# HerreraKrachTeichmann/NJODE

Hardware: AMD Instinct MI355X
Metric: paths/sec (training step) on 20k Black-Scholes, 100 steps (higher is better)
Workload: dtype f32; 1 GPU; BlackScholes 20000 paths/GPU x 100 grid steps, every rank's paths as one batch, hidden_size=10, 3x(50,50) tanh nets, dropout 0.1, train step = plan+fwd+bwd+Adam; global_batch=20000, n_obs_rows=199470, euler_steps_per_batch=1820212, params=10071, parallelism=dp1

## Files before the change

njode_amd/csrc/njode_mfma.h:

```cpp
#pragma once
#include "njode_kernels.h"

namespace njode {

typedef float f32x4 __attribute__((ext_vector_type(4)));

NJ_DEV f32x4 mfma4(float a, float b, f32x4 c) {
  return __builtin_amdgcn_mfma_f32_16x16x4f32(a, b, c, 0, 0, 0);
}

typedef unsigned u32x2 __attribute__((ext_vector_type(2)));
NJ_DEV f32x4 mfma1(float a, float b, f32x4 c) {
  return __builtin_amdgcn_mfma_f32_4x4x1f32(a, b, c, 0, 0, 0);
}
NJ_DEV float edge_reduce(float p0, float p1) {
  const u32x2 s = __builtin_amdgcn_permlane16_swap(__float_as_uint(p0), __float_as_uint(p1), false, false);
  const float t = __uint_as_float(s[0]) + __uint_as_float(s[1]);
  const u32x2 w = __builtin_amdgcn_permlane32_swap(__float_as_uint(t), __float_as_uint(t), false, false);
  return __uint_as_float(w[0]) + __uint_as_float(w[1]);
}
template <int W> struct EdgeRows {
  static constexpr int R = (W % 16 == 1 || W % 16 == 2) ? W % 16 : 0;
  static constexpr int TILE = R ? W / 16 : -1;
};
// ... 140 lines not shown
    float v = act_f<ACT>(acc[q / 4][q % 4]);
    if constexpr (DROP) v = ((keep >> q) & 1) ? v * inv_keep : 0.0f;
    av[q] = v;
  }
  constexpr int QB = W / 4, GB = W % 4;
  av[QB] = g == GB ? 1.0f : av[QB];
}
template <class C, bool DROP>
NJ_DEV void hidden_from_acc(const f32x4 (&acc)[MF<C>::MT1], float (&av)[MF<C>::Q1], uint32_t keep,
                            float inv_keep, int g) {
  hidden_from_acc_g<MF<C>::MT1, MF<C>::Q1, MF<C>::W, C::ACT, DROP>(acc, av, keep, inv_keep, g);
}

template <class C, bool DROP>
NJ_DEV void hidden_from_acc_draw(const f32x4 (&acc)[MF<C>::MT1], float (&av)[MF<C>::Q1], uint32_t& s,
                                 uint32_t thr16, float inv_keep, int g) {
  constexpr int Q1 = MF<C>::Q1;
#pragma unroll
  for (int q = 0; q < Q1; q += 2) {
    float v0 = act_f<C::ACT>(acc[q / 4][q % 4]);
    float v1 = q + 1 < Q1 ? act_f<C::ACT>(acc[(q + 1) / 4][(q + 1) % 4]) : 0.0f;
    if constexpr (DROP) {
      s ^= s << 13; s ^= s >> 17; s ^= s << 5;
      v0 = (s & 0xffffu) >= thr16 ? v0 * inv_keep : 0.0f;
      v1 = (s >> 16) >= thr16 ? v1 * inv_keep : 0.0f;
    }
    av[q] = v0;
    if (q + 1 < Q1) av[q + 1] = v1;
  }
  constexpr int QB = MF<C>::W / 4, GB = MF<C>::W % 4;
  av[QB] = g == GB ? 1.0f : av[QB];
}

template <class C, bool DROP, bool TAIL>
NJ_DEV void ode_fwd_single(const KArgs& a, int lane, int wave, int n_waves, int tile0, int tile1) {
  using M = MF<C>;
  const int g = lane >> 4, c = lane & 15;
  float A1[M::MT1][M::Q0], A2[M::MT1][M::Q1], A3[M::MTH][M::Q1];
#pragma unroll
  for (int mt = 0; mt < M::MT1; ++mt) {
#pragma unroll
    for (int q = 0; q < M::Q0; ++q) A1[mt][q] = a.frag[(M::F1 + mt * M::Q0 + q) * 64 + lane];
#pragma unroll
    for (int q = 0; q < M::Q1; ++q) A2[mt][q] = a.frag[(M::F2 + mt * M::Q1 + q) * 64 + lane];
  }
#pragma unroll
  for (int mt = 0; mt < M::MTH; ++mt)
#pragma unroll
    for (int q = 0; q < M::Q1; ++q) A3[mt][q] = a.frag[(M::F3 + mt * M::Q1 + q) * 64 + lane];

  const bool SAVE = !TAIL && a.save_traj != 0;
  const int n_items = TAIL ? a.B : a.n_obs;
  const int n_tiles = tile1 - tile0;
  float* const trash = a.trash + lane * C::H;
  for (int round = 0; round * n_waves < n_tiles; ++round) {
    const int rel = snake_tile(round, wave, n_waves);
    if (rel >= n_tiles) continue;
    const int tile = tile0 + rel;
    const int j = tile * 16 + c;
    const bool valid = j < n_items;
    Item<C> it;
    it.template load<TAIL>(a, j, valid);
    const float* h0 = it.h0(a);
    float h[M::QH];
#pragma unroll
    for (int q = 0; q < M::QH; ++q) {
// ... 424 lines not shown
```

njode_amd/csrc/njode_mfma_rows.h:

```cpp
#pragma once
#include "njode_mfma.h"

namespace njode {

template <int IN_, int OUT_, int W_> struct MS {
  static constexpr int IN = IN_, OUT = OUT_, W = W_;
  static constexpr int Q0 = (IN + 1 + 3) / 4, Q1 = (W + 1 + 3) / 4;
  static constexpr int QO = (OUT + 3) / 4, QW = (W + 3) / 4, QI = (IN + 3) / 4;
  static constexpr int MT1 = (W + 15) / 16, MTO = (OUT + 15) / 16, MTI = (IN + 15) / 16;
  static constexpr int NT1 = (W + 1 + 15) / 16, NT0 = (IN + 1 + 15) / 16;
  static constexpr int F1 = 0, F2 = F1 + MT1 * Q0, F3 = F2 + MT1 * Q1, NFWD = F3 + MTO * Q1;
  static constexpr int B3 = NFWD, B2 = B3 + MT1 * QO, B1 = B2 + MT1 * QW, NALL = B1 + MTI * QW;
  static constexpr int ET = EdgeRows<W>::TILE, ER = EdgeRows<W>::R;
  static constexpr int G2M = ER ? ET : MT1, G2N = ER ? ET : NT1;
};

template <class NL, class S>
NJ_DEV void pack_net_value(const float* __restrict__ Pn, float* __restrict__ frag, int idx) {
  if (idx >= S::NALL * 64) return;
  const int f = idx >> 6, l = idx & 63, g = l >> 4, c = l & 15;
  const float *W1 = Pn + NL::woff(0), *b1 = Pn + NL::boff(0), *W2 = Pn + NL::woff(1),
              *b2 = Pn + NL::boff(1), *W3 = Pn + NL::woff(2), *b3 = Pn + NL::boff(2);
  float v = 0.0f;
  if (f < S::F2) {
// ... 32 lines not shown
      for (int q = 0; q < S::Q0; ++q) A1[mt][q] = frag[(S::F1 + mt * S::Q0 + q) * 64 + l];
#pragma unroll
      for (int q = 0; q < S::Q1; ++q) A2[mt][q] = frag[(S::F2 + mt * S::Q1 + q) * 64 + l];
    }
    const int l3 = S::OUT == 1 ? (lane & 48) : lane;
#pragma unroll
    for (int mt = 0; mt < S::MTO; ++mt)
#pragma unroll
      for (int q = 0; q < S::Q1; ++q) A3[mt][q] = frag[(S::F3 + mt * S::Q1 + q) * 64 + l3];
  }
  NJ_DEV float r3(int q) const { return A3[0][q]; }
  NJ_DEV void begin() const {}
  NJ_DEV float a1(int mt, int q) const { return A1[mt][q]; }
  NJ_DEV float a2(int mt, int q) const { return A2[mt][q]; }
  NJ_DEV float a3(int mt, int q) const { return A3[mt][q]; }
  NJ_DEV float e1(int q) const { return A1[S::ET < 0 ? 0 : S::ET][q]; }
  NJ_DEV float e2(int q) const { return A2[S::ET < 0 ? 0 : S::ET][q]; }
};
template <class S> struct LdsFrags {
  lfp base;
  lfp cur;
  int de;
  int dr;
  NJ_DEV void init(lfp img, int lane) {
    base = img + lane;
    cur = base;
    de = edge_lane(lane) - lane;
    dr = (lane & 48) - lane;
  }
  NJ_DEV float r3(int q) const { return cur[(S::F3 + q) * 64 + dr]; }
  static NJ_DEV void stage(lfp img, const float* frag, int tid, int nthreads) {
    for (int i = tid; i < S::NALL * 64; i += nthreads) img[i] = frag[i];
  }
  NJ_DEV void begin() {
    unsigned v = (unsigned)(unsigned long long)base;
    asm volatile("" : "+v"(v));
    cur = (lfp)(unsigned long long)v;
  }
  NJ_DEV float a1(int mt, int q) const { return cur[(S::F1 + mt * S::Q0 + q) * 64]; }
  NJ_DEV float a2(int mt, int q) const { return cur[(S::F2 + mt * S::Q1 + q) * 64]; }
  NJ_DEV float a3(int mt, int q) const { return cur[(S::F3 + mt * S::Q1 + q) * 64]; }
  NJ_DEV float b3(int mt, int q) const { return cur[(S::B3 + mt * S::QO + q) * 64]; }
  NJ_DEV float b2(int mt, int q) const { return cur[(S::B2 + mt * S::QW + q) * 64]; }
  NJ_DEV float b1(int mt, int q) const { return cur[(S::B1 + mt * S::QW + q) * 64]; }
  NJ_DEV float e1(int q) const { return cur[(S::F1 + S::ET * S::Q0 + q) * 64 + de]; }
  NJ_DEV float e2(int q) const { return cur[(S::F2 + S::ET * S::Q1 + q) * 64 + de]; }
  NJ_DEV float eb3(int q) const { return cur[(S::B3 + S::ET * S::QO + q) * 64 + de]; }
  NJ_DEV float eb2(int q) const { return cur[(S::B2 + S::ET * S::QW + q) * 64 + de]; }
};
template <class S> struct GradTiles {
  f32x4 G3[S::MTO][S::NT1], G2[S::G2M][S::G2N], GM[2], GN[2], G1[S::MT1][S::NT0];
  NJ_DEV void zero() {
    const f32x4 z = {0.f, 0.f, 0.f, 0.f};
    GM[0] = GM[1] = GN[0] = GN[1] = z;
#pragma unroll
    for (int i = 0; i < S::MTO; ++i)
#pragma unroll
      for (int n = 0; n < S::NT1; ++n) G3[i][n] = z;
#pragma unroll
    for (int i = 0; i < S::G2M; ++i)
#pragma unroll
      for (int n = 0; n < S::G2N; ++n) G2[i][n] = z;
#pragma unroll
    for (int i = 0; i < S::MT1; ++i) {
#pragma unroll
      for (int n = 0; n < S::NT0; ++n) G1[i][n] = z;
// ... 8 lines not shown
      for (int nt = 0; nt < S::NT1; ++nt) f(G3[mt][nt], i++);
#pragma unroll
    for (int mt = 0; mt < S::G2M; ++mt)
#pragma unroll
      for (int nt = 0; nt < S::G2N; ++nt) f(G2[mt][nt], i++);
    if constexpr (S::ER != 0) {
      f(GM[0], i++);
      f(GN[0], i++);
    }
#pragma unroll
    for (int mt = 0; mt < S::MT1; ++mt)
#pragma unroll
      for (int nt = 0; nt < S::NT0; ++nt) f(G1[mt][nt], i++);
  }
  NJ_DEV bool reduce_block(lfp lds, int wv, int lane) {
    f32x4 __attribute__((address_space(3)))* red = (f32x4 __attribute__((address_space(3)))*)lds;
    if constexpr (S::ER != 0) {
      const f32x4 z = {0.f, 0.f, 0.f, 0.f};
      GM[0] += GM[1];
      GN[0] += GN[1];
      GM[1] = GN[1] = z;
    }
    __syncthreads();
    if (wv > 0) for_tiles([&](f32x4& t, int i) { red[((wv - 1) * NG + i) * 64 + lane] = t; });
    __syncthreads();
    if (wv != 0) return false;
    for_tiles([&](f32x4& t, int i) {
      t += red[(0 * NG + i) * 64 + lane];
      t += red[(1 * NG + i) * 64 + lane];
      t += red[(2 * NG + i) * 64 + lane];
    });
    return true;
  }
  template <class NL> NJ_DEV void flush(float* slab, int g, int c) const {
    float *W1 = slab + NL::woff(0), *b1 = slab + NL::boff(0), *W2 = slab + NL::woff(1),
          *b2 = slab + NL::boff(1), *W3 = slab + NL::woff(2), *b3 = slab + NL::boff(2);
#pragma unroll
    for (int mt = 0; mt < S::G2M; ++mt)
#pragma unroll
      for (int r = 0; r < 4; ++r) {
        const int uo = 16 * mt + 4 * g + r;
        if (uo < S::W) {
#pragma unroll
          for (int nt = 0; nt < S::G2N; ++nt) {
            const int ui = 16 * nt + c;
            if (ui < S::W) W2[uo * S::W + ui] = G2[mt][nt][r];
            else if (ui == S::W) b2[uo] = G2[mt][nt][r];
          }
        }
      }
    if constexpr (S::ER != 0) {
      const int lane = 16 * g + c;
      const f32x4 gm = GM[0] + GM[1], gn = GN[0] + GN[1];
#pragma unroll
      for (int i = 0; i < S::ER; ++i) {
        const int uo = 16 * S::ET + i;
        if (lane < S::W) W2[uo * S::W + lane] = gm[i];
        else if (lane == S::W) b2[uo] = gm[i];
      }
      if (lane < 16 * S::ET) {
#pragma unroll
        for (int i = 0; i < 4; ++i) {
          const int ui = 16 * S::ET + i;
          if (ui < S::W) W2[lane * S::W + ui] = gn[i];
          else if (ui == S::W) b2[lane] = gn[i];
        }
// ... 14 lines not shown
        }
      }
    if constexpr (S::OUT == 1) {
#pragma unroll
      for (int q = 0; q < S::Q1; ++q) {
        float v = G3[0][q / 4][q % 4];
#pragma unroll
        for (int o = 8; o > 0; o >>= 1) v += __shfl_xor(v, o);
        const int ui = 4 * q + g;
        if (c == 0) {
          if (ui < S::W) W3[ui] = v;
          else if (ui == S::W) b3[0] = v;
        }
      }
      return;
    }
#pragma unroll
    for (int mt = 0; mt < S::MTO; ++mt)
#pragma unroll
      for (int r = 0; r < 4; ++r) {
        const int uo = 16 * mt + 4 * g + r;
        if (uo < S::OUT) {
#pragma unroll
          for (int nt = 0; nt < S::NT1; ++nt) {
            const int ui = 16 * nt + c;
            if (ui < S::W) W3[uo * S::W + ui] = G3[mt][nt][r];
            else if (ui == S::W) b3[uo] = G3[mt][nt][r];
          }
        }
      }
  }
};

template <class S, int ACT, bool DROP, class FP>
NJ_DEV void mnet_fwd(FP& F, const float (&b0)[S::Q0], float (&a1)[S::Q1],
                     float (&a2)[S::Q1], f32x4 (&out)[S::MTO], uint32_t k1, uint32_t k2,
                     float inv_keep, int g) {
  const f32x4 z = {0.f, 0.f, 0.f, 0.f};
  f32x4 acc[S::MT1];
  F.begin();
#pragma unroll
  for (int mt = 0; mt < S::MT1; ++mt) acc[mt] = z;
#pragma unroll
  for (int q = 0; q < S::Q0; ++q)
#pragma unroll
    for (int mt = 0; mt < S::MT1; ++mt)
      acc[mt] = mt == S::ET ? mfma1(F.e1(q), b0[q], acc[mt]) : mfma4(F.a1(mt, q), b0[q], acc[mt]);
  if constexpr (S::ER != 0) acc[S::ET] = edge_tile<S::ER>(acc[S::ET], g);
  hidden_from_acc_g<S::MT1, S::Q1, S::W, ACT, DROP>(acc, a1, k1, inv_keep, g);
#pragma unroll
  for (int mt = 0; mt < S::MT1; ++mt) acc[mt] = z;
#pragma unroll
  for (int q = 0; q < S::Q1; ++q)
#pragma unroll
    for (int mt = 0; mt < S::MT1; ++mt)
      acc[mt] = mt == S::ET ? mfma1(F.e2(q), a1[q], acc[mt]) : mfma4(F.a2(mt, q), a1[q], acc[mt]);
  if constexpr (S::ER != 0) acc[S::ET] = edge_tile<S::ER>(acc[S::ET], g);
  hidden_from_acc_g<S::MT1, S::Q1, S::W, ACT, DROP>(acc, a2, k2, inv_keep, g);
  if constexpr (S::OUT == 1) {
    float p0 = 0.0f, p1 = 0.0f;
#pragma unroll
    for (int q = 0; q < S::Q1; q += 2) {
      p0 = fmaf(F.r3(q), a2[q], p0);
      if (q + 1 < S::Q1) p1 = fmaf(F.r3(q + 1), a2[q + 1], p1);
    }
    const float p = p0 + p1;
    out[0] = f32x4{edge_reduce(p, p), 0.0f, 0.0f, 0.0f};
    return;
  }
#pragma unroll
  for (int mt = 0; mt < S::MTO; ++mt) out[mt] = z;
#pragma unroll
  for (int q = 0; q < S::Q1; ++q)
#pragma unroll
    for (int mt = 0; mt < S::MTO; ++mt) out[mt] = mfma4(F.a3(mt, q), a2[q], out[mt]);
}

template <class S, int ACT, bool DROP, bool DIN, class FP, int ROWS = IMG_ROWS>
NJ_DEV void mnet_bwd(FP& Bf, GradTiles<S>& G, lfp img_d, lfp img_a,
                     const float (&dout)[S::QO], const float (&b0)[S::Q0],
                     const float (&a1)[S::Q1], const float (&a2)[S::Q1], uint32_t k1,
                     uint32_t k2, float inv_keep, float keepf, f32x4 (&din)[DIN ? S::MTI : 1],
                     int g, int c) {
  static_assert(16 * S::NT1 <= ROWS && 16 * S::NT0 <= ROWS && 16 * S::MTO <= ROWS &&
                    16 * S::MT1 <= ROWS,
                "dW staging images hold at most ROWS units");
  const f32x4 z = {0.f, 0.f, 0.f, 0.f};
  f32x4 acc[S::MT1];
  Bf.begin();
  if constexpr (S::OUT == 1) {
    const float d0 = g == 0 ? dout[0] : 0.0f;
    const float dyc = edge_reduce(d0, d0);
#pragma unroll
    for (int mt = 0; mt < S::MT1; ++mt) acc[mt] = z;
#pragma unroll
    for (int q = 0; q < S::Q1; ++q) {
      G.G3[0][q / 4][q % 4] = fmaf(dyc, a2[q], G.G3[0][q / 4][q % 4]);
      if (q < S::QW) {
        const float w = Bf.r3(q);
        acc[q / 4][q % 4] = (4 * q + 3 < S::W || 4 * q + g < S::W) ? w * dyc : 0.0f;
      }
    }
  } else {
    img_write<S::QO>(img_d, dout, g, c);
    img_write<S::Q1>(img_a, a2, g, c);
    wave_lds_sync();
    dw_accumulate<S::MTO, S::NT1>(img_d, img_a, G.G3, g, c);
#pragma unroll
    for (int mt = 0; mt < S::MT1; ++mt) acc[mt] = z;
#pragma unroll
    for (int q = 0; q < S::QO; ++q)
#pragma unroll
      for (int mt = 0; mt < S::MT1; ++mt)
        acc[mt] = mt == S::ET ? mfma1(Bf.eb3(q), dout[q], acc[mt]) : mfma4(Bf.b3(mt, q), dout[q], acc[mt]);
    if constexpr (S::ER != 0) acc[S::ET] = edge_tile<S::ER>(acc[S::ET], g);
  }
  float d2[S::QW];
  hidden_delta_g<S::MT1, S::Q1, S::QW, ACT, DROP>(acc, a2, d2, k2, inv_keep, keepf);
  wave_lds_sync();
  img_write<S::QW>(img_d, d2, g, c);
  img_write<S::Q1>(img_a, a1, g, c);
  wave_lds_sync();
  if constexpr (S::ER != 0) dw_accumulate_edge<S::G2M>(img_d, img_a, G.G2, G.GM, G.GN, 16 * g + c, g, c);
  else dw_accumulate<S::G2M, S::G2N>(img_d, img_a, G.G2, g, c);
#pragma unroll
  for (int mt = 0; mt < S::MT1; ++mt) acc[mt] = z;
#pragma unroll
  for (int q = 0; q < S::QW; ++q)
#pragma unroll
    for (int mt = 0; mt < S::MT1; ++mt)
      acc[mt] = mt == S::ET ? mfma1(Bf.eb2(q), d2[q], acc[mt]) : mfma4(Bf.b2(mt, q), d2[q], acc[mt]);
  if constexpr (S::ER != 0) acc[S::ET] = edge_tile<S::ER>(acc[S::ET], g);
  float d1[S::QW];
  hidden_delta_g<S::MT1, S::Q1, S::QW, ACT, DROP>(acc, a1, d1, k1, inv_keep, keepf);
  wave_lds_sync();
  img_write<S::QW>(img_d, d1, g, c);
  img_write<S::Q0>(img_a, b0, g, c);
  wave_lds_sync();
  dw_accumulate<S::MT1, S::NT0>(img_d, img_a, G.G1, g, c);
  if constexpr (DIN) {
#pragma unroll
    for (int mt = 0; mt < S::MTI; ++mt) din[mt] = z;
#pragma unroll
    for (int q = 0; q < S::QW; ++q)
#pragma unroll
      for (int mt = 0; mt < S::MTI; ++mt) din[mt] = mfma4(Bf.b1(mt, q), d1[q], din[mt]);
  }
  wave_lds_sync();
}

template <bool DROP> NJ_DEV void row_keep_bits(const KArgs& a, unsigned long long gid, uint32_t tkey,
                                               uint32_t net, int g, int nq, uint32_t& k1,
                                               uint32_t& k2) {
  k1 = k2 = 0;
  if constexpr (DROP) {
    uint32_t st = drop_state(a.dc, (uint32_t)gid, (uint32_t)(gid >> 32) + 0x5bd1e995u * (g + 1),
                             tkey, net);
    k1 = keep_bits<16>(st, a.dc.thr16);
    k2 = keep_bits<16>(st, a.dc.thr16);
  }
  (void)nq;
}

template <int Q, int N> NJ_DEV float by_group(const float (&v)[N], int g) {
  const float e0 = 4 * Q + 0 < N ? v[4 * Q + 0 < N ? 4 * Q + 0 : 0] : 0.0f;
  const float e1 = 4 * Q + 1 < N ? v[4 * Q + 1 < N ? 4 * Q + 1 : 0] : 0.0f;
  const float e2 = 4 * Q + 2 < N ? v[4 * Q + 2 < N ? 4 * Q + 2 : 0] : 0.0f;
  const float e3 = 4 * Q + 3 < N ? v[4 * Q + 3 < N ? 4 * Q + 3 : 0] : 0.0f;
  return g == 0 ? e0 : (g == 1 ? e1 : (g == 2 ? e2 : e3));
}

template <int NQ, int N, int Q = 0>
NJ_DEV void fill_by_group(float (&dq)[NQ], const float (&v)[N], int g) {
  if constexpr (Q < NQ) {
    dq[Q] = by_group<Q, N>(v, g);
    fill_by_group<NQ, N, Q + 1>(dq, v, g);
  }
}

template <class C> struct EncS { using type = MS<C::ENC_IN, C::H, C::W>; };
template <class C> struct DecS { using type = MS<C::H, C::DO, C::W>; };

template <class C, class S>
NJ_DEV void enc_input(const float* xp, float (&b0)[S::Q0], int g) {
#pragma unroll
  for (int q = 0; q < S::Q0; ++q) {
    const int u = 4 * q + g;
    const float xv = xp[u < C::D ? u : 0];
    b0[q] = u < C::D ? tanh_f(xv) : (u == C::D ? 1.0f : 0.0f);
  }
}
template <class C> NJ_DEV float enc_residual(const float* xp, int u) {
  if constexpr (C::ENC_CASE == 1) {
    return xp[u % C::D];
  } else if constexpr (C::ENC_CASE == 2) {
    constexpr int mult = C::D / C::H;
    float s = 0.0f;
#pragma unroll
    for (int cc = 0; cc < mult; ++cc) s += xp[cc * C::H + (u < C::H ? u : 0)];
    return s * (1.0f / mult);
  } else {
    return 0.0f;
  }
}

template <class C, bool DROP>
__global__ void __launch_bounds__(64) k_encode_rows_mfma(KArgs a) {
  using S = typename EncS<C>::type;
  const int lane = threadIdx.x, g = lane >> 4, c = lane & 15;
  FwdFrags<S> F;
  F.load(a.frag_enc, lane);
  const int total = a.n_obs + a.B;
  const int n_tiles = (total + 15) / 16;
  float* const trash = a.trash + lane * C::H;
  for (int tile = blockIdx.x; tile < n_tiles; tile += gridDim.x) {
    const int t0 = tile * 16 + c;
    const bool valid = t0 < total;
    const int tid = valid ? t0 : 0;
    const bool is_row = tid < a.n_obs;
    const int b = is_row ? a.obs_idx[tid] : tid - a.n_obs;
    const float* xp = is_row ? a.X + (size_t)tid * C::D : a.start_X + (size_t)b * C::D;
    float b0[S::Q0], a1[S::Q1], a2[S::Q1];
    enc_input<C, S>(xp, b0, g);
    uint32_t k1, k2;
    row_keep_bits<DROP>(a, a.gid0 + b, is_row ? (uint32_t)a.k_jump[a.t_of_row[tid]] : TKEY_START,
                        NET_ENC, g, S::Q1, k1, k2);
    f32x4 out[S::MTO];
    mnet_fwd<S, C::ACT, DROP>(F, b0, a1, a2, out, k1, k2, a.dc.inv_keep, g);
    float* dstrow = valid ? (is_row ? a.h0row + (size_t)tid * C::H : a.h0start + (size_t)b * C::H)
                          : trash;
#pragma unroll
    for (int q = 0; q < S::QO; ++q) {
      const int u = 4 * q + g;
      const float v = out[q / 4][q % 4] + enc_residual<C>(xp, u < C::H ? u : 0);
      float* dst = u < C::H ? dstrow + u : trash;
      *dst = v;
    }
  }
}

template <class C, class S>
NJ_DEV void dec_input(const float* hp, float (&b0)[S::Q0], int g) {
#pragma unroll
  for (int q = 0; q < S::Q0; ++q) {
    const int u = 4 * q + g;
    const float hv = hp[u < C::H ? u : 0];
    b0[q] = u < C::H ? tanh_f(hv) : (u == C::H ? 1.0f : 0.0f);
  }
}
template <class C, class S>
NJ_DEV void dec_collect(lfp img, const f32x4 (&out)[S::MTO], const float* hp, float (&y)[C::DO],
                        int g, int c) {
  if constexpr (C::DO == 1) {
    float v = out[0][0];
    if constexpr (C::DEC_CASE == 1) {
      v += hp[0];
    } else if constexpr (C::DEC_CASE == 2) {
      float s = 0.0f;
#pragma unroll
      for (int cc = 0; cc < C::H; ++cc) s += hp[cc];
      v += s * (1.0f / C::H);
// ... 13 lines not shown
      v += hp[u % C::H];
    } else if constexpr (C::DEC_CASE == 2) {
      constexpr int mult = C::H / C::DO;
      float s = 0.0f;
#pragma unroll
      for (int cc = 0; cc < mult; ++cc) s += hp[cc * C::DO + u];
      v += s * (1.0f / mult);
    }
    y[u] = v;
  }
  wave_lds_sync();
}

template <class C, bool DROP>
__global__ void __launch_bounds__(64) k_jump_rows_mfma(KArgs a) {
  using S = typename DecS<C>::type;
  static_assert(C::DO <= 16, "row kernels hold the full readout vector per lane");
  __shared__ __attribute__((aligned(16))) float lds_raw[IMG_FLOATS];
  lfp img = (lfp)lds_raw;
  const int lane = threadIdx.x, g = lane >> 4, c = lane & 15;
  FwdFrags<S> F;
  F.load(a.frag_dec, lane);
  const int n_tiles = (a.n_obs + 15) / 16;
  for (int tile = blockIdx.x; tile < n_tiles; tile += gridDim.x) {
    const int r0 = tile * 16 + c;
    const bool valid = r0 < a.n_obs;
    const int r = valid ? r0 : 0;
    const int b = a.obs_idx[r];
    const unsigned long long gid = a.gid0 + b;
    const uint32_t tkey = (uint32_t)a.k_jump[a.t_of_row[r]];
    const float *he = a.h_end + (size_t)r * C::H, *h0 = a.h0row + (size_t)r * C::H;
    float b0[S::Q0], a1[S::Q1], a2[S::Q1], y[C::DO], ybj[C::DO], x[C::D], mask[C::D];
    f32x4 out[S::MTO];
    uint32_t k1, k2;
    dec_input<C, S>(he, b0, g);
    row_keep_bits<DROP>(a, gid, tkey, NET_DEC_BJ, g, S::Q1, k1, k2);
    mnet_fwd<S, C::ACT, DROP>(F, b0, a1, a2, out, k1, k2, a.dc.inv_keep, g);
    dec_collect<C, S>(img, out, he, ybj, g, c);
    dec_input<C, S>(h0, b0, g);
    row_keep_bits<DROP>(a, gid, tkey, NET_DEC, g, S::Q1, k1, k2);
    mnet_fwd<S, C::ACT, DROP>(F, b0, a1, a2, out, k1, k2, a.dc.inv_keep, g);
    dec_collect<C, S>(img, out, h0, y, g, c);
    load_vec(a.X + (size_t)r * C::D, x);
#pragma unroll
    for (int i = 0; i < C::D; ++i) mask[i] = 1.0f;
    float dy[C::DO], dybj[C::DO];
    const float scale = a.inv_batch * __builtin_amdgcn_rcpf((float)a.n_obs_ot[b]);
    const float term = loss_row<C>(x, mask, y, ybj, a.weight, a.loss_easy, scale, dy, dybj);
    if (valid && g == 0) a.loss_terms[r] = term;
  }
}

template <class C, class S>
NJ_DEV void dec_input_grad(const f32x4 (&din)[S::MTI], const float (&b0)[S::Q0],
                           const float (&dyv)[C::DO], float* dst, float* trash, int g) {
#pragma unroll
  for (int q = 0; q < S::QI; ++q) {
    const int u = 4 * q + g;
    const float th = b0[q];
    float v = din[q / 4][q % 4] * (1.0f - th * th);
    if constexpr (C::DEC_CASE == 1) {
#pragma unroll
      for (int jj = 0; jj < C::DO; ++jj) v += (jj % C::H) == u ? dyv[jj] : 0.0f;
    } else if constexpr (C::DEC_CASE == 2) {
      constexpr int mult = C::H / C::DO;
      float e = 0.0f;
#pragma unroll
      for (int jj = 0; jj < C::DO; ++jj) e = (u % C::DO) == jj ? dyv[jj] : e;
      v += e * (1.0f / mult);
    }
    float* p = u < C::H ? dst + u : trash;
    *p = v;
  }
}

template <class C, bool DROP>
__global__ void __launch_bounds__(256, 2) k_jump_rows_bwd_mfma(KArgs a) {
  using S = typename DecS<C>::type;
  using NL = typename C::Dec;
  __shared__ __attribute__((aligned(16))) float lds_raw[4 * 2 * IMG_FLOATS + S::NALL * 64];
  const int lane = threadIdx.x & 63, wv = threadIdx.x >> 6, g = lane >> 4, c = lane & 15;
  const int wave = blockIdx.x * 4 + wv, n_waves = gridDim.x * 4;
  lfp img_d = (lfp)lds_raw + wv * 2 * IMG_FLOATS, img_a = img_d + IMG_FLOATS;
  lfp fimg = (lfp)lds_raw + 4 * 2 * IMG_FLOATS;
  LdsFrags<S>::stage(fimg, a.frag_dec, threadIdx.x, 256);
  for (int i = threadIdx.x; i < 4 * 2 * IMG_FLOATS; i += 256) lds_raw[i] = 0.0f;
  __syncthreads();
  LdsFrags<S> F;
  F.init(fimg, lane);
  LdsFrags<S>& Bf = F;
  GradTiles<S> G;
  G.zero();
  float* const trash = a.trash + threadIdx.x * C::H;
  const int n_tiles = (a.n_obs + 15) / 16;
  for (int tile = wave; tile < n_tiles; tile += n_waves) {
    const int r0 = tile * 16 + c;
    const bool valid = r0 < a.n_obs;
    const int r = valid ? r0 : 0;
    const int b = a.obs_idx[r];
    const unsigned long long gid = a.gid0 + b;
    const uint32_t tkey = (uint32_t)a.k_jump[a.t_of_row[r]];
    const float *he = a.h_end + (size_t)r * C::H, *h0 = a.h0row + (size_t)r * C::H;
    float b0[S::Q0], a1[S::Q1], a2[S::Q1], y[C::DO], ybj[C::DO], x[C::D], mask[C::D];
    float dy[C::DO], dybj[C::DO], dq[S::QO];
    f32x4 out[S::MTO], din[S::MTI];
    uint32_t kb1, kb2, k1, k2;
    float b0b[S::Q0], a1b[S::Q1], a2b[S::Q1];
    dec_input<C, S>(he, b0b, g);
    row_keep_bits<DROP>(a, gid, tkey, NET_DEC_BJ, g, S::Q1, kb1, kb2);
    mnet_fwd<S, C::ACT, DROP>(F, b0b, a1b, a2b, out, kb1, kb2, a.dc.inv_keep, g);
    dec_collect<C, S>(img_d, out, he, ybj, g, c);
    dec_input<C, S>(h0, b0, g);
    row_keep_bits<DROP>(a, gid, tkey, NET_DEC, g, S::Q1, k1, k2);
    mnet_fwd<S, C::ACT, DROP>(F, b0, a1, a2, out, k1, k2, a.dc.inv_keep, g);
    dec_collect<C, S>(img_d, out, h0, y, g, c);
    load_vec(a.X + (size_t)r * C::D, x);
#pragma unroll
    for (int i = 0; i < C::D; ++i) mask[i] = 1.0f;
    const float scale = (valid ? a.inv_batch : 0.0f) * __builtin_amdgcn_rcpf((float)a.n_obs_ot[b]);
    const float term = loss_row<C>(x, mask, y, ybj, a.weight, a.loss_easy, scale, dy, dybj);
    if (a.defer_loss && valid && g == 0) a.loss_terms[r] = term;
    fill_by_group<S::QO, C::DO>(dq, dy, g);
    mnet_bwd<S, C::ACT, DROP, true>(Bf, G, img_d, img_a, dq, b0, a1, a2, k1, k2, a.dc.inv_keep,
                                    a.keep, din, g, c);
    dec_input_grad<C, S>(din, b0, dy, valid ? a.g_h0 + (size_t)r * C::H : trash, trash, g);
    fill_by_group<S::QO, C::DO>(dq, dybj, g);
    mnet_bwd<S, C::ACT, DROP, true>(Bf, G, img_d, img_a, dq, b0b, a1b, a2b, kb1, kb2,
                                    a.dc.inv_keep, a.keep, din, g, c);
    dec_input_grad<C, S>(din, b0b, dybj, valid ? a.lam_end + (size_t)r * C::H : trash, trash, g);
  }
  static_assert(3 * GradTiles<S>::NG * 256 <= 4 * 2 * IMG_FLOATS + S::NALL * 64, "tile reduction does not fit");
  if (G.reduce_block((lfp)lds_raw, wv, lane))
    G.template flush<NL>(a.slab + (size_t)blockIdx.x * C::P + C::OFF_DEC, g, c);
}

template <class C> struct EncBwdLds {
  static constexpr int FLOATS = 4 * 2 * IMG_FLOATS + EncS<C>::type::NALL * 64;
};
template <class C, bool DROP>
NJ_DEV void encode_rows_bwd_body(const KArgs& a, float* lds_raw, int block, int n_blocks) {
  using S = typename EncS<C>::type;
  using NL = typename C::Enc;
  const int lane = threadIdx.x & 63, wv = threadIdx.x >> 6, g = lane >> 4, c = lane & 15;
  const int wave = block * 4 + wv, n_waves = n_blocks * 4;
  lfp img_d = (lfp)lds_raw + wv * 2 * IMG_FLOATS, img_a = img_d + IMG_FLOATS;
  lfp fimg = (lfp)lds_raw + 4 * 2 * IMG_FLOATS;
  LdsFrags<S>::stage(fimg, a.frag_enc, threadIdx.x, 256);
  for (int i = threadIdx.x; i < 4 * 2 * IMG_FLOATS; i += 256) lds_raw[i] = 0.0f;
  __syncthreads();
  LdsFrags<S> F;
  F.init(fimg, lane);
  LdsFrags<S>& Bf = F;
  GradTiles<S> G;
  G.zero();
  const int total = a.n_obs + a.B;
  const int n_tiles = (total + 15) / 16;
  for (int tile = wave; tile < n_tiles; tile += n_waves) {
    const int t0 = tile * 16 + c;
    const bool valid = t0 < total;
    const int tid = valid ? t0 : 0;
    const bool is_row = tid < a.n_obs;
    const int b = is_row ? a.obs_idx[tid] : tid - a.n_obs;
    const float* xp = is_row ? a.X + (size_t)tid * C::D : a.start_X + (size_t)b * C::D;
    const int nxt = is_row ? a.item_next[tid] : a.first_row[b];
    const int nx = nxt >= 0 ? nxt : 0, rr = is_row ? tid : 0;
    float gh[S::QO];
#pragma unroll
    for (int q = 0; q < S::QO; ++q) {
      const int u = 4 * q + g, uu = u < C::H ? u : 0;
      const float l = a.lam_start[(size_t)nx * C::H + uu];
      const float p = a.g_h0[(size_t)rr * C::H + uu];
      gh[q] = (valid && u < C::H) ? ((nxt >= 0 ? l : 0.0f) + (is_row ? p : 0.0f)) : 0.0f;
    }
    float b0[S::Q0], a1[S::Q1], a2[S::Q1];
    enc_input<C, S>(xp, b0, g);
    uint32_t k1, k2;
    row_keep_bits<DROP>(a, a.gid0 + b, is_row ? (uint32_t)a.k_jump[a.t_of_row[tid]] : TKEY_START,
                        NET_ENC, g, S::Q1, k1, k2);
    f32x4 out[S::MTO], din[1];
    mnet_fwd<S, C::ACT, DROP>(F, b0, a1, a2, out, k1, k2, a.dc.inv_keep, g);
    mnet_bwd<S, C::ACT, DROP, false>(Bf, G, img_d, img_a, gh, b0, a1, a2, k1, k2, a.dc.inv_keep,
                                     a.keep, din, g, c);
  }
  static_assert(3 * GradTiles<S>::NG * 256 <= 4 * 2 * IMG_FLOATS + S::NALL * 64, "tile reduction does not fit");
  if (G.reduce_block((lfp)lds_raw, wv, lane))
    G.template flush<NL>(a.slab + (size_t)block * C::P + C::OFF_ENC, g, c);
}
template <class C, bool DROP>
__global__ void __launch_bounds__(256, 2) k_encode_rows_bwd_mfma(KArgs a) {
  __shared__ __attribute__((aligned(16))) float lds_raw[EncBwdLds<C>::FLOATS];
  encode_rows_bwd_body<C, DROP>(a, lds_raw, (int)blockIdx.x, (int)gridDim.x);
}

}
```

Measured before the change: 23.10 million paths/s.

## Mark dropped units with negative zero, split block gradient reduction across waves

Row encoder and decoder nets no longer precompute keep bitmasks. Forward dropout draws the xorshift state inline and marks dropped units as -0.0, and backward recovers the mask from that sign pattern, so the keep-bit generation and its register use go away. The block gradient reduction now spreads tile ownership across all four waves, each reducing and flushing its own tiles, instead of wave 0 doing all of it. Weight fragments are staged into LDS with 16-byte vector loads. The RNG draw order changes, so the dropout masks differ from the previous scheme, and the design relies on an activation never being exactly -0.0 when kept.

```diff
diff --git a/njode_amd/csrc/njode_mfma.h b/njode_amd/csrc/njode_mfma.h
--- a/njode_amd/csrc/njode_mfma.h
+++ b/njode_amd/csrc/njode_mfma.h
@@ -196,6 +196,46 @@
   av[QB] = g == GB ? 1.0f : av[QB];
 }
 
+template <int MT1, int Q1, int W, int ACT, bool DROP, int NDRAW>
+NJ_DEV void hidden_from_acc_mark(const f32x4 (&acc)[MT1], float (&av)[Q1], uint32_t& s, uint32_t thr16,
+                                 float inv_keep, int g) {
+  static_assert(Q1 <= NDRAW, "a layer's units draw from its own words");
+#pragma unroll
+  for (int q = 0; q < Q1; q += 2) {
+    float v0 = act_f<ACT>(acc[q / 4][q % 4]);
+    float v1 = q + 1 < Q1 ? act_f<ACT>(acc[(q + 1) / 4][(q + 1) % 4]) : 0.0f;
+    if constexpr (DROP) {
+      s ^= s << 13; s ^= s >> 17; s ^= s << 5;
+      v0 = (s & 0xffffu) >= thr16 ? v0 * inv_keep : -0.0f;
+      v1 = (s >> 16) >= thr16 ? v1 * inv_keep : -0.0f;
+    }
+    av[q] = v0;
+    if (q + 1 < Q1) av[q + 1] = v1;
+  }
+  if constexpr (DROP) {
+#pragma unroll
+    for (int u = (Q1 + 1) / 2 * 2; u < NDRAW; u += 2) { s ^= s << 13; s ^= s >> 17; s ^= s << 5; }
+  }
+  constexpr int QB = W / 4, GB = W % 4;
+  av[QB] = g == GB ? 1.0f : av[QB];
+}
+template <int MT1, int Q1, int QW, int ACT, bool DROP>
+NJ_DEV void hidden_delta_mark(const f32x4 (&acc)[MT1], const float (&av)[Q1], float (&dv)[QW],
+                              float inv_keep, float keepf) {
+#pragma unroll
+  for (int q = 0; q < QW; ++q) {
+    const float gsum = acc[q / 4][q % 4];
+    if constexpr (DROP) {
+      float f;
+      if constexpr (ACT == ACT_TANH) f = fmaf(av[q] * av[q], -keepf, inv_keep);
+      else f = inv_keep * dact_f<ACT>(av[q] * keepf);
+      dv[q] = __float_as_uint(av[q]) != 0x80000000u ? gsum * f : 0.0f;
+    } else {
+      dv[q] = gsum * dact_f<ACT>(av[q]);
+    }
+  }
+}
+
 template <class C, bool DROP, bool TAIL>
 NJ_DEV void ode_fwd_single(const KArgs& a, int lane, int wave, int n_waves, int tile0, int tile1) {
   using M = MF<C>;
diff --git a/njode_amd/csrc/njode_mfma_rows.h b/njode_amd/csrc/njode_mfma_rows.h
--- a/njode_amd/csrc/njode_mfma_rows.h
+++ b/njode_amd/csrc/njode_mfma_rows.h
@@ -88,6 +88,25 @@
   static NJ_DEV void stage(lfp img, const float* frag, int tid, int nthreads) {
     for (int i = tid; i < S::NALL * 64; i += nthreads) img[i] = frag[i];
   }
+  template <int NZ> static NJ_DEV void stage16(lfp img, lfp zero, const float* frag, int tid) {
+    typedef f32x4 __attribute__((address_space(3))) * lv4;
+    constexpr int N4 = S::NALL * 16, PER = (N4 + 255) / 256;
+    static_assert(NZ % 4 == 0, "whole 16-byte vectors");
+    const f32x4* src = (const f32x4*)frag;
+    const f32x4 z = {0.f, 0.f, 0.f, 0.f};
+    f32x4 v[PER];
+#pragma unroll
+    for (int j = 0; j < PER; ++j) {
+      const int i = tid + j * 256;
+      v[j] = (j + 1 < PER || N4 % 256 == 0 || i < N4) ? src[i < N4 ? i : 0] : z;
+    }
+    for (int i = tid; i < NZ / 4; i += 256) ((lv4)zero)[i] = z;
+#pragma unroll
+    for (int j = 0; j < PER; ++j) {
+      const int i = tid + j * 256;
+      if (j + 1 < PER || N4 % 256 == 0 || i < N4) ((lv4)img)[i] = v[j];
+    }
+  }
   NJ_DEV void begin() {
     unsigned v = (unsigned)(unsigned long long)base;
     asm volatile("" : "+v"(v));
@@ -162,6 +181,101 @@
     });
     return true;
   }
+  static constexpr int owner(int i) { return (S::OUT == 1 && i < S::MTO * S::NT1) ? 0 : i * 4 / NG; }
+  NJ_DEV void reduce_quarters(lfp lds, int wv, int lane) {
+    f32x4 __attribute__((address_space(3)))* red = (f32x4 __attribute__((address_space(3)))*)lds;
+    if constexpr (S::ER != 0) {
+      const f32x4 z = {0.f, 0.f, 0.f, 0.f};
+      GM[0] += GM[1];
+      GN[0] += GN[1];
+      GM[1] = GN[1] = z;
+    }
+    __syncthreads();
+    for_tiles([&](f32x4& t, int i) {
+      const int o = owner(i);
+      if (wv != o) red[((wv < o ? wv : wv - 1) * NG + i) * 64 + lane] = t;
+    });
+    __syncthreads();
+    for_tiles([&](f32x4& t, int i) {
+      const int o = owner(i);
+      if (wv == o) {
+        f32x4 s = o == 0 ? t : red[(0 * NG + i) * 64 + lane];
+#pragma unroll
+        for (int w = 1; w < 4; ++w) s += w == o ? t : red[((w < o ? w : w - 1) * NG + i) * 64 + lane];
+        t = s;
+      }
+    });
+  }
+  template <class NL> NJ_DEV void flush_owned(float* slab, int wv, int g, int c) const {
+    float *W1 = slab + NL::woff(0), *b1 = slab + NL::boff(0), *W2 = slab + NL::woff(1),
+          *b2 = slab + NL::boff(1), *W3 = slab + NL::woff(2), *b3 = slab + NL::boff(2);
+    auto store = [&](const f32x4& t, float* Wm, float* bv, int mt, int nt, int NO, int NI)
+        __attribute__((always_inline)) {
+#pragma unroll
+      for (int r = 0; r < 4; ++r) {
+        const int uo = 16 * mt + 4 * g + r, ui = 16 * nt + c;
+        if (uo < NO) {
+          if (ui < NI) Wm[uo * NI + ui] = t[r];
+          else if (ui == NI) bv[uo] = t[r];
+        }
+      }
+    };
+    int i = 0;
+    if constexpr (S::OUT == 1) {
+      if (wv == 0) {
+#pragma unroll
+        for (int q = 0; q < S::Q1; ++q) {
+          float v = G3[0][q / 4][q % 4];
+#pragma unroll
+          for (int o = 8; o > 0; o >>= 1) v += __shfl_xor(v, o);
+          const int ui = 4 * q + g;
+          if (c == 0) {
+            if (ui < S::W) W3[ui] = v;
+            else if (ui == S::W) b3[0] = v;
+          }
+        }
+      }
+      i += S::MTO * S::NT1;
+    } else {
+#pragma unroll
+      for (int mt = 0; mt < S::MTO; ++mt)
+#pragma unroll
+        for (int nt = 0; nt < S::NT1; ++nt, ++i)
+          if (wv == owner(i)) store(G3[mt][nt], W3, b3, mt, nt, S::OUT, S::W);
+    }
+#pragma unroll
+    for (int mt = 0; mt < S::G2M; ++mt)
+#pragma unroll
+      for (int nt = 0; nt < S::G2N; ++nt, ++i)
+        if (wv == owner(i)) store(G2[mt][nt], W2, b2, mt, nt, S::W, S::W);
+    if constexpr (S::ER != 0) {
+      const int lane = 16 * g + c;
+      const f32x4 gm = GM[0] + GM[1], gn = GN[0] + GN[1];
+      if (wv == owner(i)) {
+#pragma unroll
+        for (int e = 0; e < S::ER; ++e) {
+          const int uo = 16 * S::ET + e;
+          if (lane < S::W) W2[uo * S::W + lane] = gm[e];
+          else if (lane == S::W) b2[uo] = gm[e];
+        }
+      }
+      ++i;
+      if (wv == owner(i) && lane < 16 * S::ET) {
+#pragma unroll
+        for (int e = 0; e < 4; ++e) {
+          const int ui = 16 * S::ET + e;
+          if (ui < S::W) W2[lane * S::W + ui] = gn[e];
+          else if (ui == S::W) b2[lane] = gn[e];
+        }
+      }
+      ++i;
+    }
+#pragma unroll
+    for (int mt = 0; mt < S::MT1; ++mt)
+#pragma unroll
+      for (int nt = 0; nt < S::NT0; ++nt, ++i)
+        if (wv == owner(i)) store(G1[mt][nt], W1, b1, mt, nt, S::W, S::IN);
+  }
   template <class NL> NJ_DEV void flush(float* slab, int g, int c) const {
     float *W1 = slab + NL::woff(0), *b1 = slab + NL::boff(0), *W2 = slab + NL::woff(1),
           *b2 = slab + NL::boff(1), *W3 = slab + NL::woff(2), *b3 = slab + NL::boff(2);
@@ -242,56 +356,62 @@
   }
 };
 
+template <class S, class FP, class HID>
+NJ_DEV void mnet_fwd_with(FP& F, const float (&b0)[S::Q0], float (&a1)[S::Q1],
+                          float (&a2)[S::Q1], f32x4 (&out)[S::MTO], HID hid, int g) {
+  const f32x4 z = {0.f, 0.f, 0.f, 0.f};
+  f32x4 acc[S::MT1];
+  F.begin();
+#pragma unroll
+  for (int mt = 0; mt < S::MT1; ++mt) acc[mt] = z;
+#pragma unroll
+  for (int q = 0; q < S::Q0; ++q)
+#pragma unroll
+    for (int mt = 0; mt < S::MT1; ++mt)
+      acc[mt] = mt == S::ET ? mfma1(F.e1(q), b0[q], acc[mt]) : mfma4(F.a1(mt, q), b0[q], acc[mt]);
+  if constexpr (S::ER != 0) acc[S::ET] = edge_tile<S::ER>(acc[S::ET], g);
+  hid(acc, a1, 0);
+#pragma unroll
+  for (int mt = 0; mt < S::MT1; ++mt) acc[mt] = z;
+#pragma unroll
+  for (int q = 0; q < S::Q1; ++q)
+#pragma unroll
+    for (int mt = 0; mt < S::MT1; ++mt)
+      acc[mt] = mt == S::ET ? mfma1(F.e2(q), a1[q], acc[mt]) : mfma4(F.a2(mt, q), a1[q], acc[mt]);
+  if constexpr (S::ER != 0) acc[S::ET] = edge_tile<S::ER>(acc[S::ET], g);
+  hid(acc, a2, 1);
+  if constexpr (S::OUT == 1) {
+    float p0 = 0.0f, p1 = 0.0f;
+#pragma unroll
+    for (int q = 0; q < S::Q1; q += 2) {
+      p0 = fmaf(F.r3(q), a2[q], p0);
+      if (q + 1 < S::Q1) p1 = fmaf(F.r3(q + 1), a2[q + 1], p1);
+    }
+    const float p = p0 + p1;
+    out[0] = f32x4{edge_reduce(p, p), 0.0f, 0.0f, 0.0f};
+    return;
+  }
+#pragma unroll
+  for (int mt = 0; mt < S::MTO; ++mt) out[mt] = z;
+#pragma unroll
+  for (int q = 0; q < S::Q1; ++q)
+#pragma unroll
+    for (int mt = 0; mt < S::MTO; ++mt) out[mt] = mfma4(F.a3(mt, q), a2[q], out[mt]);
+}
 template <class S, int ACT, bool DROP, class FP>
 NJ_DEV void mnet_fwd(FP& F, const float (&b0)[S::Q0], float (&a1)[S::Q1],
                      float (&a2)[S::Q1], f32x4 (&out)[S::MTO], uint32_t k1, uint32_t k2,
                      float inv_keep, int g) {
-  const f32x4 z = {0.f, 0.f, 0.f, 0.f};
-  f32x4 acc[S::MT1];
-  F.begin();
-#pragma unroll
-  for (int mt = 0; mt < S::MT1; ++mt) acc[mt] = z;
-#pragma unroll
-  for (int q = 0; q < S::Q0; ++q)
-#pragma unroll
-    for (int mt = 0; mt < S::MT1; ++mt)
-      acc[mt] = mt == S::ET ? mfma1(F.e1(q), b0[q], acc[mt]) : mfma4(F.a1(mt, q), b0[q], acc[mt]);
-  if constexpr (S::ER != 0) acc[S::ET] = edge_tile<S::ER>(acc[S::ET], g);
-  hidden_from_acc_g<S::MT1, S::Q1, S::W, ACT, DROP>(acc, a1, k1, inv_keep, g);
-#pragma unroll
-  for (int mt = 0; mt < S::MT1; ++mt) acc[mt] = z;
-#pragma unroll
-  for (int q = 0; q < S::Q1; ++q)
-#pragma unroll
-    for (int mt = 0; mt < S::MT1; ++mt)
-      acc[mt] = mt == S::ET ? mfma1(F.e2(q), a1[q], acc[mt]) : mfma4(F.a2(mt, q), a1[q], acc[mt]);
-  if constexpr (S::ER != 0) acc[S::ET] = edge_tile<S::ER>(acc[S::ET], g);
-  hidden_from_acc_g<S::MT1, S::Q1, S::W, ACT, DROP>(acc, a2, k2, inv_keep, g);
-  if constexpr (S::OUT == 1) {
-    float p0 = 0.0f, p1 = 0.0f;
-#pragma unroll
-    for (int q = 0; q < S::Q1; q += 2) {
-      p0 = fmaf(F.r3(q), a2[q], p0);
-      if (q + 1 < S::Q1) p1 = fmaf(F.r3(q + 1), a2[q + 1], p1);
-    }
-    const float p = p0 + p1;
-    out[0] = f32x4{edge_reduce(p, p), 0.0f, 0.0f, 0.0f};
-    return;
-  }
-#pragma unroll
-  for (int mt = 0; mt < S::MTO; ++mt) out[mt] = z;
-#pragma unroll
-  for (int q = 0; q < S::Q1; ++q)
-#pragma unroll
-    for (int mt = 0; mt < S::MTO; ++mt) out[mt] = mfma4(F.a3(mt, q), a2[q], out[mt]);
-}
-
-template <class S, int ACT, bool DROP, bool DIN, class FP, int ROWS = IMG_ROWS>
-NJ_DEV void mnet_bwd(FP& Bf, GradTiles<S>& G, lfp img_d, lfp img_a,
-                     const float (&dout)[S::QO], const float (&b0)[S::Q0],
-                     const float (&a1)[S::Q1], const float (&a2)[S::Q1], uint32_t k1,
-                     uint32_t k2, float inv_keep, float keepf, f32x4 (&din)[DIN ? S::MTI : 1],
-                     int g, int c) {
+  mnet_fwd_with<S>(F, b0, a1, a2, out, [&](const f32x4 (&acc)[S::MT1], float (&av)[S::Q1], int layer) __attribute__((always_inline)) {
+    hidden_from_acc_g<S::MT1, S::Q1, S::W, ACT, DROP>(acc, av, layer ? k2 : k1, inv_keep, g);
+  }, g);
+}
+
+template <class S, bool DIN, int ROWS, class FP, class DEL>
+NJ_DEV void mnet_bwd_with(FP& Bf, GradTiles<S>& G, lfp img_d, lfp img_a,
+                          const float (&dout)[S::QO], const float (&b0)[S::Q0],
+                          const float (&a1)[S::Q1], const float (&a2)[S::Q1], DEL del,
+                          f32x4 (&din)[DIN ? S::MTI : 1], int g, int c) {
   static_assert(16 * S::NT1 <= ROWS && 16 * S::NT0 <= ROWS && 16 * S::MTO <= ROWS &&
                     16 * S::MT1 <= ROWS,
                 "dW staging images hold at most ROWS units");
@@ -326,7 +446,7 @@
     if constexpr (S::ER != 0) acc[S::ET] = edge_tile<S::ER>(acc[S::ET], g);
   }
   float d2[S::QW];
-  hidden_delta_g<S::MT1, S::Q1, S::QW, ACT, DROP>(acc, a2, d2, k2, inv_keep, keepf);
+  del(acc, a2, d2, 1);
   wave_lds_sync();
   img_write<S::QW>(img_d, d2, g, c);
   img_write<S::Q1>(img_a, a1, g, c);
@@ -342,7 +462,7 @@
       acc[mt] = mt == S::ET ? mfma1(Bf.eb2(q), d2[q], acc[mt]) : mfma4(Bf.b2(mt, q), d2[q], acc[mt]);
   if constexpr (S::ER != 0) acc[S::ET] = edge_tile<S::ER>(acc[S::ET], g);
   float d1[S::QW];
-  hidden_delta_g<S::MT1, S::Q1, S::QW, ACT, DROP>(acc, a1, d1, k1, inv_keep, keepf);
+  del(acc, a1, d1, 0);
   wave_lds_sync();
   img_write<S::QW>(img_d, d1, g, c);
   img_write<S::Q0>(img_a, b0, g, c);
@@ -357,6 +477,18 @@
       for (int mt = 0; mt < S::MTI; ++mt) din[mt] = mfma4(Bf.b1(mt, q), d1[q], din[mt]);
   }
   wave_lds_sync();
+}
+template <class S, int ACT, bool DROP, bool DIN, class FP, int ROWS = IMG_ROWS>
+NJ_DEV void mnet_bwd(FP& Bf, GradTiles<S>& G, lfp img_d, lfp img_a,
+                     const float (&dout)[S::QO], const float (&b0)[S::Q0],
+                     const float (&a1)[S::Q1], const float (&a2)[S::Q1], uint32_t k1,
+                     uint32_t k2, float inv_keep, float keepf, f32x4 (&din)[DIN ? S::MTI : 1],
+                     int g, int c) {
+  mnet_bwd_with<S, DIN, ROWS>(Bf, G, img_d, img_a, dout, b0, a1, a2,
+                              [&](const f32x4 (&acc)[S::MT1], const float (&av)[S::Q1], float (&dv)[S::QW],
+                                  int layer) __attribute__((always_inline)) {
+    hidden_delta_g<S::MT1, S::Q1, S::QW, ACT, DROP>(acc, av, dv, layer ? k2 : k1, inv_keep, keepf);
+  }, din, g, c);
 }
 
 template <bool DROP> NJ_DEV void row_keep_bits(const KArgs& a, unsigned long long gid, uint32_t tkey,
@@ -370,6 +502,52 @@
     k2 = keep_bits<16>(st, a.dc.thr16);
   }
   (void)nq;
+}
+
+#ifndef NJ_ROW_MARK
+#define NJ_ROW_MARK 1
+#endif
+#ifndef NJ_ROW_EDGES
+#define NJ_ROW_EDGES 1
+#endif
+struct RowKeep { uint32_t k1, k2; };
+
+template <class S, int ACT, bool DROP, class FP>
+NJ_DEV void mnet_fwd_row(FP& F, const KArgs& a, unsigned long long gid, uint32_t tkey, uint32_t net,
+                         const float (&b0)[S::Q0], float (&a1)[S::Q1], float (&a2)[S::Q1],
+                         f32x4 (&out)[S::MTO], RowKeep& k, int g) {
+#if NJ_ROW_MARK
+  k.k1 = k.k2 = 0;
+  uint32_t st = 0;
+  if constexpr (DROP)
+    st = drop_state(a.dc, (uint32_t)gid, (uint32_t)(gid >> 32) + 0x5bd1e995u * (g + 1), tkey, net);
+  const uint32_t thr16 = a.dc.thr16;
+  const float inv_keep = a.dc.inv_keep;
+  mnet_fwd_with<S>(F, b0, a1, a2, out,
+                   [&](const f32x4 (&acc)[S::MT1], float (&av)[S::Q1], int layer) __attribute__((always_inline)) {
+    if (layer == 0) hidden_from_acc_mark<S::MT1, S::Q1, S::W, ACT, DROP, 16>(acc, av, st, thr16, inv_keep, g);
+    else hidden_from_acc_mark<S::MT1, S::Q1, S::W, ACT, DROP, (S::Q1 + 1) / 2 * 2>(acc, av, st, thr16, inv_keep, g);
+  }, g);
+#else
+  row_keep_bits<DROP>(a, gid, tkey, net, g, S::Q1, k.k1, k.k2);
+  mnet_fwd<S, ACT, DROP>(F, b0, a1, a2, out, k.k1, k.k2, a.dc.inv_keep, g);
+#endif
+}
+template <class S, int ACT, bool DROP, bool DIN, class FP>
+NJ_DEV void mnet_bwd_row(FP& Bf, GradTiles<S>& G, lfp img_d, lfp img_a, const float (&dout)[S::QO],
+                         const float (&b0)[S::Q0], const float (&a1)[S::Q1], const float (&a2)[S::Q1],
+                         const RowKeep& k, float inv_keep, float keepf, f32x4 (&din)[DIN ? S::MTI : 1],
+                         int g, int c) {
+#if NJ_ROW_MARK
+  (void)k;
+  mnet_bwd_with<S, DIN, IMG_ROWS>(Bf, G, img_d, img_a, dout, b0, a1, a2,
+                                  [&](const f32x4 (&acc)[S::MT1], const float (&av)[S::Q1], float (&dv)[S::QW],
+                                      int) __attribute__((always_inline)) {
+    hidden_delta_mark<S::MT1, S::Q1, S::QW, ACT, DROP>(acc, av, dv, inv_keep, keepf);
+  }, din, g, c);
+#else
+  mnet_bwd<S, ACT, DROP, DIN>(Bf, G, img_d, img_a, dout, b0, a1, a2, k.k1, k.k2, inv_keep, keepf, din, g, c);
+#endif
 }
 
 template <int Q, int N> NJ_DEV float by_group(const float (&v)[N], int g) {
@@ -432,11 +610,10 @@
     const float* xp = is_row ? a.X + (size_t)tid * C::D : a.start_X + (size_t)b * C::D;
     float b0[S::Q0], a1[S::Q1], a2[S::Q1];
     enc_input<C, S>(xp, b0, g);
-    uint32_t k1, k2;
-    row_keep_bits<DROP>(a, a.gid0 + b, is_row ? (uint32_t)a.k_jump[a.t_of_row[tid]] : TKEY_START,
-                        NET_ENC, g, S::Q1, k1, k2);
+    RowKeep kp;
     f32x4 out[S::MTO];
-    mnet_fwd<S, C::ACT, DROP>(F, b0, a1, a2, out, k1, k2, a.dc.inv_keep, g);
+    mnet_fwd_row<S, C::ACT, DROP>(F, a, a.gid0 + b, is_row ? (uint32_t)a.k_jump[a.t_of_row[tid]] : TKEY_START,
+                                  NET_ENC, b0, a1, a2, out, kp, g);
     float* dstrow = valid ? (is_row ? a.h0row + (size_t)tid * C::H : a.h0start + (size_t)b * C::H)
                           : trash;
 #pragma unroll
@@ -516,14 +693,12 @@
     const float *he = a.h_end + (size_t)r * C::H, *h0 = a.h0row + (size_t)r * C::H;
     float b0[S::Q0], a1[S::Q1], a2[S::Q1], y[C::DO], ybj[C::DO], x[C::D], mask[C::D];
     f32x4 out[S::MTO];
-    uint32_t k1, k2;
+    RowKeep kp;
     dec_input<C, S>(he, b0, g);
-    row_keep_bits<DROP>(a, gid, tkey, NET_DEC_BJ, g, S::Q1, k1, k2);
-    mnet_fwd<S, C::ACT, DROP>(F, b0, a1, a2, out, k1, k2, a.dc.inv_keep, g);
+    mnet_fwd_row<S, C::ACT, DROP>(F, a, gid, tkey, NET_DEC_BJ, b0, a1, a2, out, kp, g);
     dec_collect<C, S>(img, out, he, ybj, g, c);
     dec_input<C, S>(h0, b0, g);
-    row_keep_bits<DROP>(a, gid, tkey, NET_DEC, g, S::Q1, k1, k2);
-    mnet_fwd<S, C::ACT, DROP>(F, b0, a1, a2, out, k1, k2, a.dc.inv_keep, g);
+    mnet_fwd_row<S, C::ACT, DROP>(F, a, gid, tkey, NET_DEC, b0, a1, a2, out, kp, g);
     dec_collect<C, S>(img, out, h0, y, g, c);
     load_vec(a.X + (size_t)r * C::D, x);
 #pragma unroll
@@ -567,8 +742,12 @@
   const int wave = blockIdx.x * 4 + wv, n_waves = gridDim.x * 4;
   lfp img_d = (lfp)lds_raw + wv * 2 * IMG_FLOATS, img_a = img_d + IMG_FLOATS;
   lfp fimg = (lfp)lds_raw + 4 * 2 * IMG_FLOATS;
+#if NJ_ROW_EDGES
+  LdsFrags<S>::template stage16<4 * 2 * IMG_FLOATS>(fimg, (lfp)lds_raw, a.frag_dec, threadIdx.x);
+#else
   LdsFrags<S>::stage(fimg, a.frag_dec, threadIdx.x, 256);
   for (int i = threadIdx.x; i < 4 * 2 * IMG_FLOATS; i += 256) lds_raw[i] = 0.0f;
+#endif
   __syncthreads();
   LdsFrags<S> F;
   F.init(fimg, lane);
@@ -588,15 +767,13 @@
     float b0[S::Q0], a1[S::Q1], a2[S::Q1], y[C::DO], ybj[C::DO], x[C::D], mask[C::D];
     float dy[C::DO], dybj[C::DO], dq[S::QO];
     f32x4 out[S::MTO], din[S::MTI];
-    uint32_t kb1, kb2, k1, k2;
+    RowKeep kb, kp;
     float b0b[S::Q0], a1b[S::Q1], a2b[S::Q1];
     dec_input<C, S>(he, b0b, g);
-    row_keep_bits<DROP>(a, gid, tkey, NET_DEC_BJ, g, S::Q1, kb1, kb2);
-    mnet_fwd<S, C::ACT, DROP>(F, b0b, a1b, a2b, out, kb1, kb2, a.dc.inv_keep, g);
+    mnet_fwd_row<S, C::ACT, DROP>(F, a, gid, tkey, NET_DEC_BJ, b0b, a1b, a2b, out, kb, g);
     dec_collect<C, S>(img_d, out, he, ybj, g, c);
     dec_input<C, S>(h0, b0, g);
-    row_keep_bits<DROP>(a, gid, tkey, NET_DEC, g, S::Q1, k1, k2);
-    mnet_fwd<S, C::ACT, DROP>(F, b0, a1, a2, out, k1, k2, a.dc.inv_keep, g);
+    mnet_fwd_row<S, C::ACT, DROP>(F, a, gid, tkey, NET_DEC, b0, a1, a2, out, kp, g);
     dec_collect<C, S>(img_d, out, h0, y, g, c);
     load_vec(a.X + (size_t)r * C::D, x);
 #pragma unroll
@@ -605,17 +782,22 @@
     const float term = loss_row<C>(x, mask, y, ybj, a.weight, a.loss_easy, scale, dy, dybj);
     if (a.defer_loss && valid && g == 0) a.loss_terms[r] = term;
     fill_by_group<S::QO, C::DO>(dq, dy, g);
-    mnet_bwd<S, C::ACT, DROP, true>(Bf, G, img_d, img_a, dq, b0, a1, a2, k1, k2, a.dc.inv_keep,
-                                    a.keep, din, g, c);
+    mnet_bwd_row<S, C::ACT, DROP, true>(Bf, G, img_d, img_a, dq, b0, a1, a2, kp, a.dc.inv_keep,
+                                        a.keep, din, g, c);
     dec_input_grad<C, S>(din, b0, dy, valid ? a.g_h0 + (size_t)r * C::H : trash, trash, g);
     fill_by_group<S::QO, C::DO>(dq, dybj, g);
-    mnet_bwd<S, C::ACT, DROP, true>(Bf, G, img_d, img_a, dq, b0b, a1b, a2b, kb1, kb2,
-                                    a.dc.inv_keep, a.keep, din, g, c);
+    mnet_bwd_row<S, C::ACT, DROP, true>(Bf, G, img_d, img_a, dq, b0b, a1b, a2b, kb,
+                                        a.dc.inv_keep, a.keep, din, g, c);
     dec_input_grad<C, S>(din, b0b, dybj, valid ? a.lam_end + (size_t)r * C::H : trash, trash, g);
   }
   static_assert(3 * GradTiles<S>::NG * 256 <= 4 * 2 * IMG_FLOATS + S::NALL * 64, "tile reduction does not fit");
+#if NJ_ROW_EDGES
+  G.reduce_quarters((lfp)lds_raw, wv, lane);
+  G.template flush_owned<NL>(a.slab + (size_t)blockIdx.x * C::P + C::OFF_DEC, wv, g, c);
+#else
   if (G.reduce_block((lfp)lds_raw, wv, lane))
     G.template flush<NL>(a.slab + (size_t)blockIdx.x * C::P + C::OFF_DEC, g, c);
+#endif
 }
 
 template <class C> struct EncBwdLds {
@@ -629,8 +811,12 @@
   const int wave = block * 4 + wv, n_waves = n_blocks * 4;
   lfp img_d = (lfp)lds_raw + wv * 2 * IMG_FLOATS, img_a = img_d + IMG_FLOATS;
   lfp fimg = (lfp)lds_raw + 4 * 2 * IMG_FLOATS;
+#if NJ_ROW_EDGES
+  LdsFrags<S>::template stage16<4 * 2 * IMG_FLOATS>(fimg, (lfp)lds_raw, a.frag_enc, threadIdx.x);
+#else
   LdsFrags<S>::stage(fimg, a.frag_enc, threadIdx.x, 256);
   for (int i = threadIdx.x; i < 4 * 2 * IMG_FLOATS; i += 256) lds_raw[i] = 0.0f;
+#endif
   __syncthreads();
   LdsFrags<S> F;
   F.init(fimg, lane);
@@ -658,17 +844,21 @@
     }
     float b0[S::Q0], a1[S::Q1], a2[S::Q1];
     enc_input<C, S>(xp, b0, g);
-    uint32_t k1, k2;
-    row_keep_bits<DROP>(a, a.gid0 + b, is_row ? (uint32_t)a.k_jump[a.t_of_row[tid]] : TKEY_START,
-                        NET_ENC, g, S::Q1, k1, k2);
+    RowKeep kp;
     f32x4 out[S::MTO], din[1];
-    mnet_fwd<S, C::ACT, DROP>(F, b0, a1, a2, out, k1, k2, a.dc.inv_keep, g);
-    mnet_bwd<S, C::ACT, DROP, false>(Bf, G, img_d, img_a, gh, b0, a1, a2, k1, k2, a.dc.inv_keep,
-                                     a.keep, din, g, c);
+    mnet_fwd_row<S, C::ACT, DROP>(F, a, a.gid0 + b, is_row ? (uint32_t)a.k_jump[a.t_of_row[tid]] : TKEY_START,
+                                  NET_ENC, b0, a1, a2, out, kp, g);
+    mnet_bwd_row<S, C::ACT, DROP, false>(Bf, G, img_d, img_a, gh, b0, a1, a2, kp, a.dc.inv_keep,
+                                         a.keep, din, g, c);
   }
   static_assert(3 * GradTiles<S>::NG * 256 <= 4 * 2 * IMG_FLOATS + S::NALL * 64, "tile reduction does not fit");
+#if NJ_ROW_EDGES
+  G.reduce_quarters((lfp)lds_raw, wv, lane);
+  G.template flush_owned<NL>(a.slab + (size_t)block * C::P + C::OFF_ENC, wv, g, c);
+#else
   if (G.reduce_block((lfp)lds_raw, wv, lane))
     G.template flush<NL>(a.slab + (size_t)block * C::P + C::OFF_ENC, g, c);
+#endif
 }
 template <class C, bool DROP>
 __global__ void __launch_bounds__(256, 2) k_encode_rows_bwd_mfma(KArgs a) {
```

Result: faster. 23.45 million paths/s (median of 6 runs) (+1.5%).
